# davipatti/abdpymc

Measured on NVIDIA B200. Metric: logp+grad evals/s (10k individuals, joint logp + 17-dim gradient, per chain), higher is better.
Workload: dtype f64

## Files before the change

abdpymc_b200/csrc/abd_b200.cu:

```cuda
#include <algorithm>
#include <atomic>
#include <chrono>
#include <cmath>
#include <cstdio>
#include <cstdlib>
#include <cstring>
#include <map>
#include <string>
#include <type_traits>
#include <vector>

#include <cuda_runtime.h>

#include "../../include/abd_b200.h"
#include "abd_device.cuh"

using namespace abd;

namespace {

thread_local std::string g_err;

int fail(int code, const std::string& msg) {
  g_err = msg;
// ... 181 lines not shown
    if (gap[r] < 0 || gap[r] >= G) return fail(ABD_ERR_INVALID, "gap index out of range");
    rp[(size_t)ind[r] + 1]++;
  }
  for (int n = 0; n < N; ++n) rp[n + 1] += rp[n];
  std::vector<int64_t> order((size_t)R);
  {
    std::vector<int> cur(rp.begin(), rp.end() - 1);
    for (int64_t r = 0; r < R; ++r) order[(size_t)cur[ind[r]]++] = r;
  }
  for (int n = 0; n < N; ++n)
    std::stable_sort(order.begin() + rp[n], order.begin() + rp[n + 1],
                     [&](int64_t p, int64_t q) { return gap[p] < gap[q]; });
  std::vector<double> xs((size_t)R + 2, 0.0), ods((size_t)R + 2, 0.0);
  std::vector<uint32_t> meta((size_t)R + 4, 0u);
  std::vector<uint32_t> rowcell((size_t)R + 4, 0u), cmeta;
  std::vector<int>& cp = h->h_cp[a];
  cp.assign((size_t)N + 1, 0);
  std::vector<int> perm((size_t)R);
  for (int64_t k = 0; k < R; ++k) {
    const int64_t r = order[(size_t)k];
    perm[(size_t)k] = (int)r;
    xs[(size_t)k] = x[r];
    ods[(size_t)k] = od[r];
    const uint32_t m = ((uint32_t)ind[r] << gap_bits) | (uint32_t)gap[r];
    meta[(size_t)k] = m;
    if (cmeta.empty() || cmeta.back() != m) {
      cmeta.push_back(m);
      cp[(size_t)ind[r] + 1]++;
    }
    rowcell[(size_t)k] = (uint32_t)cmeta.size() - 1;
  }
  for (int n = 0; n < N; ++n) cp[n + 1] += cp[n];
  cmeta.resize(cmeta.size() + 4, 0u);
  int rc;
  int* d_rp;
  double *d_x, *d_od;
  uint32_t *d_meta, *d_rowcell, *d_cmeta;
  if ((rc = upload(h, &d_rp, rp))) return rc;
  if ((rc = upload(h, &d_x, xs))) return rc;
  if ((rc = upload(h, &d_od, ods))) return rc;
  if ((rc = upload(h, &d_meta, meta))) return rc;
  if ((rc = upload(h, &d_rowcell, rowcell))) return rc;
  if ((rc = upload(h, &d_cmeta, cmeta))) return rc;
  {
    int* d_perm;
    if ((rc = upload(h, &d_perm, perm))) return rc;
    h->dc.rowperm[a] = d_perm;
  }
  h->dc.rcx[a] = nullptr;
  if (h->fx) {
    std::vector<uint32_t> rcx((size_t)R + 4, 0u);
    for (int64_t k = 0; k < R; ++k) {
      const double* lv = h->desc.hd.xlev;
      const int xi = (int)(std::lower_bound(lv, lv + h->desc.hd.n_xlev, xs[(size_t)k]) - lv);
      rcx[(size_t)k] = (rowcell[(size_t)k] << 5) | (uint32_t)xi;
    }
    uint32_t* d_rcx;
    if ((rc = upload(h, &d_rcx, rcx))) return rc;
    h->dc.rcx[a] = d_rcx;
  }
  h->dc.rp[a] = d_rp;
  h->dc.x[a] = d_x;
  h->dc.od[a] = d_od;
  h->dc.meta[a] = d_meta;
  h->dc.rowcell[a] = d_rowcell;
  h->dc.cmeta[a] = d_cmeta;
  return ABD_OK;
}

int get_tiling(abd_handle* h, int want, abd_handle::Tiling** out) {
  auto it = h->tilings.find(want);
  if (it == h->tilings.end()) {
    const int N = h->N;
    const std::vector<int>&rn = h->h_rp[0], &rs = h->h_rp[1];
    const double total = (double)rn[N] + (double)rs[N];
    std::vector<int> ti{0};
    int inds = 0;
    for (int n = 0; n < N; ++n) {
      const double before = (double)rn[n] + (double)rs[n];
      const double target = total * (double)ti.size() / (double)want;
      if (inds > 0 && (inds == kTileMaxInds || (before >= target && (int)ti.size() < want))) {
        ti.push_back(n);
        inds = 0;
      }
      ++inds;
    }
    ti.push_back(N);
    abd_handle::Tiling t;
    t.ntiles = (int)ti.size() - 1;
    const std::vector<int>&cn = h->h_cp[0], &cs = h->h_cp[1];
    auto span = [](int lo, int hi, int al) { return ((hi + al - 1) & ~(al - 1)) - (lo & ~(al - 1)); };
    for (int k = 0; k < t.ntiles; ++k) {
      const int a = ti[k], b = ti[k + 1];
      t.cap_n = std::max(t.cap_n, span(rn[a], rn[b], 2));
      t.cap_s = std::max(t.cap_s, span(rs[a], rs[b], 2));
      t.capr_n = std::max(t.capr_n, span(rn[a], rn[b], 4));
      t.capr_s = std::max(t.capr_s, span(rs[a], rs[b], 4));
      t.capk_n = std::max(t.capk_n, span(cn[a], cn[b], 4));
      t.capk_s = std::max(t.capk_s, span(cs[a], cs[b], 4));
    }
    t.cap_n = std::max(t.cap_n, 2);
    t.cap_s = std::max(t.cap_s, 2);
    t.capr_n = std::max(t.capr_n, 4);
    t.capr_s = std::max(t.capr_s, 4);
    t.capk_n = std::max(t.capk_n, 4);
    t.capk_s = std::max(t.capk_s, 4);
    const size_t rows_b = (size_t)(t.cap_n + t.cap_s) * 8 + (size_t)(t.capr_n + t.capr_s) * 4, cells = (size_t)(t.capk_n + t.capk_s);
    t.smem = rows_b + (h->fx ? cells * (sizeof(CellValT<true, false>) + 4)
                             : cells * (sizeof(CellValT<false, false>) + 4) + (size_t)(t.cap_n + t.cap_s) * 8);
    t.smem_cp = h->fx ? rows_b + cells * (sizeof(CellValT<true, true>) + 8 + 4) : 0;
    if (t.smem_cp && t.smem_cp + 12 * 1024 > h->smem_optin) t.smem_cp = 0;
    if (t.smem + 12 * 1024 > h->smem_optin) t.smem = 0;
    if (!t.smem && !t.smem_cp)
      return fail(ABD_ERR_INVALID, "an individual tile does not fit in shared memory (too many OD rows per 128 individuals)");
    std::vector<TileDesc> desc((size_t)t.ntiles);
    for (int k = 0; k < t.ntiles; ++k) {
      const int a = ti[k], b = ti[k + 1];
      desc[(size_t)k] = TileDesc{a, b, rn[a], rn[b], rs[a], rs[b], cn[a], cn[b], cs[a], cs[b], 0, 0};
    }
    TileDesc* d_desc = nullptr;
    int rc = upload(h, &d_desc, desc);
    if (rc) return rc;
    t.d_tiles = d_desc;
    it = h->tilings.emplace(want, t).first;
  }
  *out = &it->second;
  return ABD_OK;
}

void free_chains(abd_handle* h) {
  h->chain_bufs.release();
  if (h->h_pin) cudaFreeHost(h->h_pin);
  h->h_pin = h->h_pin_dev = nullptr;
  h->cap_chains = h->pack_valid = 0;
}

int ensure_chains(abd_handle* h, int C) {
  if (C <= 0) return fail(ABD_ERR_INVALID, "n_chains must be positive");
  if (C > 65535) return fail(ABD_ERR_INVALID, "n_chains must be <= 65535");
  if (C <= h->cap_chains) return ABD_OK;
  CU(cudaStreamSynchronize(h->stream));
  const int oldC = h->cap_chains;
  const size_t gn = (size_t)h->G * h->N;
  int rc;
  DevBufs next;
  int8_t *ni, *nw;
  if ((rc = next.alloc(&ni, (size_t)C * gn)) || (rc = next.alloc(&nw, (size_t)C * h->N))) return rc;
  CU(cudaMemset(ni, 0, (size_t)C * gn));
  CU(cudaMemset(nw, 0, (size_t)C * h->N));
  if (oldC) {
    CU(cudaMemcpy(ni, h->d_iraw, (size_t)oldC * gn, cudaMemcpyDeviceToDevice));
    CU(cudaMemcpy(nw, h->d_waner, (size_t)oldC * h->N, cudaMemcpyDeviceToDevice));
  }
  free_chains(h);
  std::swap(h->chain_bufs.ptrs, next.ptrs);
  h->d_iraw = ni;
  h->d_waner = nw;
  DevBufs& b = h->chain_bufs;
  char* pk = nullptr;
  const size_t entry = with_mask(h, [](auto m) { return sizeof(PackedState<decltype(m)>); });
  if ((rc = b.alloc(&pk, (size_t)C * h->N * entry))) return rc;
  h->d_pack = pk;
  if ((rc = b.alloc(&h->d_theta, (size_t)C * 17)) || (rc = b.alloc(&h->d_p, (size_t)C * 2)) ||
      (rc = b.alloc(&h->d_sums, (size_t)C * kNSums)) || (rc = b.alloc(&h->d_out, (size_t)C * 18)) ||
      (rc = b.alloc(&h->d_ticket, (size_t)C)) || (rc = b.alloc(&h->d_aux, (size_t)C * kAuxDoubles)) ||
      (rc = b.alloc(&h->d_traj, (size_t)C * 34)) || (rc = b.alloc(&h->d_gen, (size_t)C + 1)) ||
      (rc = b.alloc(&h->d_stats, (size_t)C * 2)) || (rc = b.alloc(&h->d_queue, (size_t)C)))
    return rc;
  CU(cudaMemset(h->d_ticket, 0, (size_t)C * sizeof(unsigned)));
  CU(cudaMemset(h->d_gen, 0, ((size_t)C + 1) * sizeof(unsigned)));
  CU(cudaMallocHost((void**)&h->h_pin, (size_t)C * 40 * sizeof(double)));
  {
    void* dp = nullptr;
    if (cudaHostGetDevicePointer(&dp, h->h_pin, 0) == cudaSuccess) h->h_pin_dev = (double*)dp;
    else cudaGetLastError();
  }
  h->cap_chains = C;
  return ABD_OK;
}

constexpr int kTileRowsOneWave = 2750;
void plan_grid(const abd_handle* h, int C, int ctas_per_sm, int cpc_fixed, int one_wave_rows, int* want_tiles,
               int* chains_per_cta) {
  const double rows = (double)(h->R[0] + h->R[1]);
  const int target = h->tile_rows_override > 0 ? h->tile_rows_override : 2200;
  const int min_tiles = (h->N + kTileMaxInds - 1) / kTileMaxInds;
  const int resident = h->n_sms * ctas_per_sm;
  auto tiles_for = [&](int cpc, int* tiles_out) -> double {
    const int groups = (C + cpc - 1) / cpc;
    int tiles = std::max(min_tiles, (int)std::ceil(rows / target));
    double waves = std::ceil((double)tiles * groups / resident);
    if ((long)tiles * groups <= 6L * resident) {
      for (int w = 1; w <= 6; ++w) {
        const int t = (resident * w) / groups;
        const double limit = (w == 1 && one_wave_rows > target && h->tile_rows_override == 0) ? (double)one_wave_rows : target * 1.02;
        if (t >= min_tiles && t >= 1 && rows / t <= limit) {
          tiles = t;
          waves = w;
          break;
        }
      }
    }
    *tiles_out = std::max(1, std::min(tiles, h->N));
    return waves;
  };
  int cpc = cpc_fixed > 0 ? cpc_fixed : (C >= 64 ? 4 : (C >= 32 ? 2 : 1));
  cpc = std::min(cpc, C);
  cpc = std::min(cpc, kMaxChainsPerCta);
  int tiles;
  const double waves1 = tiles_for(cpc, &tiles);
  if (cpc_fixed == 0 && cpc == 1 && waves1 >= 3.0) {
    double best = 9.3 * waves1;
    for (int k = 2; k <= 4 && k <= C; k *= 2) {
      if (C % k) continue;
      int tk;
      const double cost = tiles_for(k, &tk) * (1.0 + 8.3 * k);
      if (cost < 0.85 * 9.3 * waves1 && cost < best) best = cost, cpc = k, tiles = tk;
    }
  }
  *want_tiles = tiles;
  *chains_per_cta = cpc;
}

template <typename M, typename XT, bool TRAJ, bool CP>
struct SumsKernel {
  using Mask = M;
  static auto fn() { return k_sums<M, XT, TRAJ, CP>; }
};

template <typename F>
auto with_sums(const abd_handle* h, bool compact, bool traj, F&& f) {
  return with_mask(h, [&](auto m) {
    using M = decltype(m);
    if (compact) return traj ? f(SumsKernel<M, uint8_t, true, true>{}) : f(SumsKernel<M, uint8_t, false, true>{});
    if (h->fx) return traj ? f(SumsKernel<M, uint8_t, true, false>{}) : f(SumsKernel<M, uint8_t, false, false>{});
    return traj ? f(SumsKernel<M, double, true, false>{}) : f(SumsKernel<M, double, false, false>{});
  });
}

template <typename K>
cudaError_t sums_smem_attr(K, int device, size_t smem) {
  static size_t configured[64] = {};
  const int d = (device >= 0 && device < 64) ? device : 0;
  const size_t want = std::max<size_t>(smem, 48 * 1024);
  if (want <= configured[d]) return cudaSuccess;
  cudaError_t e = cudaFuncSetAttribute(K::fn(), cudaFuncAttributeMaxDynamicSharedMemorySize, (int)want);
  if (e != cudaSuccess) return e;
  e = cudaFuncSetAttribute(K::fn(), cudaFuncAttributePreferredSharedMemoryCarveout, cudaSharedmemCarveoutMaxShared);
  if (e != cudaSuccess) return e;
  configured[d] = want;
  return cudaSuccess;
}

cudaError_t sums_occupancy(const abd_handle* h, bool compact, size_t smem, int* occ) {
  return with_sums(h, compact, false, [&](auto k) {
    cudaError_t e = sums_smem_attr(k, h->device, smem);
    if (e != cudaSuccess) return e;
    return cudaOccupancyMaxActiveBlocksPerMultiprocessor(occ, decltype(k)::fn(), kSumsBlock, smem);
  });
}

cudaLaunchConfig_t pdl_config(dim3 grid, dim3 block, size_t smem, cudaStream_t st, cudaLaunchAttribute* attr) {
  cudaLaunchConfig_t lc{};
  lc.gridDim = grid;
  lc.blockDim = block;
  lc.dynamicSmemBytes = smem;
  lc.stream = st;
  attr->id = cudaLaunchAttributeProgrammaticStreamSerialization;
  attr->val.programmaticStreamSerializationAllowed = 1;
  lc.attrs = attr;
  lc.numAttrs = 1;
  return lc;
}

int resident_pack(abd_handle* h, int C, const int8_t* i_raw, const int8_t* waner, cudaStream_t st, void** out) {
  *out = nullptr;
  if (i_raw != h->d_iraw || waner != h->d_waner || !h->d_pack) return ABD_OK;
  if (h->pack_valid < C) {
    if (!h->lazy_pack) return ABD_OK;
    dim3 grid((h->N + 127) / 128, C);
    with_mask(h, [&](auto m) {
      using M = decltype(m);
      k_pack<M><<<grid, 128, 0, st>>>(h->dc, h->d_iraw, h->d_waner, (PackedState<M>*)h->d_pack);
    });
    CU(cudaGetLastError());
    h->launches++;
    h->pack_valid = C;
  }
  *out = h->d_pack;
  return ABD_OK;
}

int launch_sums(abd_handle* h, int C, const double* theta, int theta_is_q, const int8_t* i_raw,
                const int8_t* waner, double* sums, const FinalizeCfg& fin, cudaStream_t st,
                const TrajCfg* traj_in = nullptr, bool sharded = false) {
  TrajCfg traj{};
  if (traj_in) traj = *traj_in;
  const ThetaInline thin = h->thin;
  h->thin.n = 0;
  const int cpc_fixed = traj.n_steps == 1 ? 1 : h->chains_per_cta_override;
  int want, cpc, rc;
  bool compact = false;
  abd_handle::Tiling* tl = nullptr;
  for (int attempt = 0; attempt < 2 * ABD_SUMS_MINB; ++attempt) {
    const int occ = ABD_SUMS_MINB - attempt / 2;
    const int one_wave_rows = (attempt & 1) ? 0 : kTileRowsOneWave;
    plan_grid(h, C, occ, cpc_fixed, one_wave_rows, &want, &cpc);
    if (traj.n_steps > 1 && cpc != 1) {
      cpc = 1;
      want = std::max((h->N + kTileMaxInds - 1) / kTileMaxInds, (h->n_sms * occ) / C);
      want = std::max(1, std::min(want, h->N));
    }
    if ((rc = get_tiling(h, want, &tl))) return rc;
    if (tl->smem && !tl->occ) {
      int o = 0;
      CU(sums_occupancy(h, false, tl->smem, &o));
      tl->occ = std::max(o, 1);
    }
    compact = false;
    if (tl->smem && tl->occ >= occ && !(h->force_compact && tl->smem_cp)) break;
    if (tl->smem_cp && !tl->occ_cp) {
      int o = 0;
      CU(sums_occupancy(h, true, tl->smem_cp, &o));
      tl->occ_cp = std::max(o, 1);
    }
    compact = tl->smem_cp != 0;
    if (compact && tl->occ_cp >= occ) break;
  }
  const int tl_occ = compact ? tl->occ_cp : tl->occ;
  if (traj.n_steps > 1) {
    if (cpc != 1 || (long)tl->ntiles * C > (long)h->n_sms * tl_occ)
      return fail(ABD_ERR_INVALID, "abd_leapfrog_dev: too many chains for one resident grid on this cohort; "
                                   "use abd_logp_dlogp_dev per step");
  }
  const size_t need = (size_t)C * tl->ntiles * kNSums;
  if (need > h->cap_partial) {
    CU(cudaStreamSynchronize(st));
    h->partial_buf.release();
    h->cap_partial = 0;
    if ((rc = h->partial_buf.alloc(&h->d_partial, need))) return rc;
    h->cap_partial = need;
  }
  SumsCfg cfg{tl->ntiles, tl->cap_n, tl->cap_s, tl->capr_n, tl->capr_s, tl->capk_n, tl->capk_s, cpc, C};
  dim3 grid(tl->ntiles, (C + cpc - 1) / cpc);
  const size_t smem = compact ? tl->smem_cp : tl->smem;
  h->last_plan[0] = tl->ntiles, h->last_plan[1] = (int)grid.y, h->last_plan[2] = cpc;
  h->last_plan[3] = (int)smem, h->last_plan[4] = compact ? 1 : 0, h->last_plan[5] = tl_occ;
  void* pack = nullptr;
  if ((rc = resident_pack(h, C, i_raw, waner, st, &pack))) return rc;
  const bool tj = traj.n_steps > 0;
  rc = with_sums(h, compact, tj, [&](auto k) -> int {
    using K = decltype(k);
    CU(sums_smem_attr(k, h->device, smem));
    cudaLaunchAttribute attr;
    cudaLaunchConfig_t lc = pdl_config(grid, dim3(kSumsBlock), smem, st, &attr);
    if (traj.n_steps > 1) {
      int occ = 0;
      CU(cudaOccupancyMaxActiveBlocksPerMultiprocessor(&occ, K::fn(), kSumsBlock, smem));
      if ((long)grid.x * grid.y > (long)occ * h->n_sms)
        return fail(ABD_ERR_INVALID, "abd_leapfrog_dev: the grid does not fit on the device at once");
      attr.id = cudaLaunchAttributeCooperative;
      attr.val.cooperative = 1;
    }
    CU(cudaLaunchKernelEx(&lc, K::fn(), h->dc, reinterpret_cast<const TileDesc*>(tl->d_tiles), cfg, theta, theta_is_q, i_raw,
                          waner, reinterpret_cast<const PackedState<typename K::Mask>*>(pack), h->d_partial, h->d_ticket, sums,
                          fin, h->d_priors, h->d_aux, traj, sharded ? h->xch : XchCfg{}, tj ? ThetaInline{} : thin));
    return ABD_OK;
  });
  if (rc) return rc;
  CU(cudaGetLastError());
  h->launches++;
  return ABD_OK;
}

int launch_gibbs(abd_handle* h, int C, const double* theta, int theta_is_q, const double* p,
                 const double* pw, int8_t* i_raw, int8_t* waner, const GibbsCfg& cfg, cudaStream_t st) {
  if (cfg.mode == ABD_GIBBS_BLOCKED) {
    if (h->mask_bits > 32 || h->dc.ch.n < 2) {
      GibbsCfg c2 = cfg;
      c2.mode = ABD_GIBBS_HEATBATH;
      return launch_gibbs(h, C, theta, theta_is_q, p, pw, i_raw, waner, c2, st);
    }
    if (!h->gibbs_blk_ctas) {
      int occ = 0;
      CU(cudaOccupancyMaxActiveBlocksPerMultiprocessor(&occ, k_gibbs_blk, kGibbsWarps * 32, 0));
      h->gibbs_blk_ctas = h->n_sms * std::max(occ, 1);
    }
    const long items = (long)C * h->N;
    const int grid = (int)std::min<long>(h->gibbs_blk_ctas, (items + kGibbsWarps - 1) / kGibbsWarps);
    CU(cudaMemsetAsync(h->d_queue, 0, (size_t)C * sizeof(unsigned), st));
    void* pack = nullptr;
    int rcp = resident_pack(h, C, i_raw, waner, st, &pack);
    if (rcp) return rcp;
    k_gibbs_blk<<<grid, kGibbsWarps * 32, 0, st>>>(h->dc, h->d_order, C, theta, theta_is_q, p, pw, i_raw, waner,
                                                   (PackedState<uint32_t>*)pack, h->d_queue, cfg);
    CU(cudaGetLastError());
    h->launches++;
    return ABD_OK;
  }
  if (!h->gibbs_ctas) {
    int occ = 0;
    CU(with_mask(h, [&](auto m) {
      return cudaOccupancyMaxActiveBlocksPerMultiprocessor(&occ, k_gibbs<decltype(m)>, kGibbsWarps * 32, 0);
    }));
    h->gibbs_ctas = h->n_sms * std::max(occ, 1);
  }
  const long items = (long)C * h->N;
  const int grid = (int)std::min<long>(h->gibbs_ctas, (items + kGibbsWarps - 1) / kGibbsWarps);
  CU(cudaMemsetAsync(h->d_queue, 0, (size_t)C * sizeof(unsigned), st));
  void* pack = nullptr;
  int rcp = resident_pack(h, C, i_raw, waner, st, &pack);
  if (rcp) return rcp;
  with_mask(h, [&](auto m) {
    using M = decltype(m);
    k_gibbs<M><<<grid, kGibbsWarps * 32, 0, st>>>(h->dc, h->d_order, C, theta, theta_is_q, p, pw, i_raw, waner,
                                                   (PackedState<M>*)pack, h->d_queue, cfg);
  });
  CU(cudaGetLastError());
  h->launches++;
  return ABD_OK;
}

int set_device(const abd_handle* h) {
  CU(cudaSetDevice(h->device));
  return ABD_OK;
}

int copy_state(abd_handle* h, void* dst, const void* src, size_t bytes, cudaMemcpyKind dir) {
  const bool h2d = dir == cudaMemcpyHostToDevice;
  const void* host = h2d ? src : dst;
  if (bytes >= (4u << 10) && (reinterpret_cast<uintptr_t>(host) & 15u) == 0) {
    cudaPointerAttributes at{};
    if (cudaPointerGetAttributes(&at, host) == cudaSuccess && at.type == cudaMemoryTypeHost && at.devicePointer) {
      const size_t n16 = bytes / 16, rem = bytes - n16 * 16;
      const int grid = (int)std::min<size_t>((size_t)h->n_sms * 4, (n16 + 255) / 256);
      k_pull<<<grid, 256, 0, h->stream>>>(reinterpret_cast<const uint4*>(h2d ? at.devicePointer : src),
                                          reinterpret_cast<uint4*>(h2d ? dst : at.devicePointer), n16, rem);
      CU(cudaGetLastError());
      h->launches++;
      return ABD_OK;
    }
    cudaGetLastError();
  }
  CU(cudaMemcpyAsync(dst, src, bytes, dir, h->stream));
  return ABD_OK;
}

int stage_state(abd_handle* h, int C, const int8_t* i_raw, const int8_t* waner) {
  const size_t gn = (size_t)h->G * h->N;
  int rc;
  h->lazy_pack = !(i_raw || waner);
  if (i_raw || waner) h->pack_valid = 0;
  if (i_raw && (rc = copy_state(h, h->d_iraw, i_raw, (size_t)C * gn, cudaMemcpyHostToDevice))) return rc;
  if (waner && (rc = copy_state(h, h->d_waner, waner, (size_t)C * h->N, cudaMemcpyHostToDevice))) return rc;
  return ABD_OK;
}

int new_handle(abd_handle** out, int device, const CohortDesc& d) {
  abd_handle* h = new abd_handle();
  h->device = device;
  if (const char* e = std::getenv("ABD_B200_COMPACT_CELLS")) h->force_compact = (e[0] == '1');
  {
    int v = 0;
    if (cudaDeviceGetAttribute(&v, cudaDevAttrMultiProcessorCount, device) == cudaSuccess && v > 0) h->n_sms = v;
    if (cudaDeviceGetAttribute(&v, cudaDevAttrMaxSharedMemoryPerBlockOptin, device) == cudaSuccess) h->smem_optin = (size_t)v;
  }
  const CacheHeader& hd = d.hd;
  h->desc = d;
  h->G = h->dc.G = hd.G;
  h->N = h->dc.N = hd.N;
  h->mask_bits = 32 << hd.wide;
  h->R[0] = hd.R[0], h->R[1] = hd.R[1];
  h->tot = Totals{hd.tot[0], hd.tot[1], hd.tot[2], hd.tot[3]};
  h->dc.ind_offset = hd.ind_offset;
  h->dc.chain_offset = 0;
  h->dc.ch.n = hd.n_chunks;
  for (int k = 0; k < 3; ++k) h->dc.ch.mask[k] = hd.chunk_mask[k], h->dc.ch.mask_hi[k] = d.mask_hi[k];
  h->fx = hd.fx != 0;
  h->dc.n_xlev = hd.n_xlev;
  int rc = ABD_OK;
  double* d_lv = nullptr;
  if (cudaStreamCreateWithFlags(&h->stream, cudaStreamNonBlocking) != cudaSuccess) rc = fail(ABD_ERR_CUDA, "cudaStreamCreate failed");
  if (!rc) rc = upload(h, &d_lv, std::vector<double>(hd.xlev, hd.xlev + kMaxXLevels));
  if (!rc) rc = upload(h, &h->d_priors, std::vector<Priors>{default_priors(hd.G)});
  if (rc) {
    abd_destroy(h);
    return rc;
  }
  h->dc.xlev = d_lv;
  *out = h;
  return ABD_OK;
}

struct CacheIo {
  FILE* f = nullptr;
  bool writing = false, ok = true;
  ~CacheIo() {
    if (f) std::fclose(f);
  }
  void raw(void* p, size_t bytes) {
    if (!ok || !bytes) return;
    ok = writing ? std::fwrite(p, 1, bytes, f) == bytes : std::fread(p, 1, bytes, f) == bytes;
    const size_t padn = (16 - bytes % 16) % 16;
    char z[16] = {};
    if (ok && padn) ok = writing ? std::fwrite(z, 1, padn, f) == padn : std::fread(z, 1, padn, f) == padn;
  }
};

template <typename T>
int cache_array(abd_handle* h, CacheIo& io, T** dptr, size_t n, std::vector<T>* keep = nullptr) {
  std::vector<T> host(n);
  if (io.writing) {
    if (n) CU(cudaMemcpy(host.data(), *dptr, n * sizeof(T), cudaMemcpyDeviceToHost));
    io.raw(host.data(), n * sizeof(T));
  } else {
    io.raw(host.data(), n * sizeof(T));
    if (!io.ok) return fail(ABD_ERR_INVALID, "cache file truncated");
    int rc = upload(h, dptr, host);
    if (rc) return rc;
    if (keep) *keep = host;
  }
  return io.ok ? ABD_OK : fail(ABD_ERR_INVALID, "cache file I/O error");
}

int cache_body(abd_handle* h, CacheIo& io) {
  const CacheHeader& hd = h->desc.hd;
  int rc;
  const size_t N = (size_t)hd.N;
  rc = with_mask(h, [&](auto m) {
    using M = decltype(m);
    M *p = (M*)h->dc.pcr, *v = (M*)h->dc.vac;
    const int r = cache_array(h, io, &p, N);
    if (r) return r;
    h->dc.pcr = p;
    const int r2 = cache_array(h, io, &v, N);
    h->dc.vac = v;
    return r2;
  });
  if (rc) return rc;
  for (int a = 0; a < 2; ++a) {
    const size_t R = (size_t)hd.R[a], K = (size_t)hd.K[a];
    int* rp = (int*)h->dc.rp[a];
    double *x = (double*)h->dc.x[a], *od = (double*)h->dc.od[a];
    uint32_t *meta = (uint32_t*)h->dc.meta[a], *rowcell = (uint32_t*)h->dc.rowcell[a], *cmeta = (uint32_t*)h->dc.cmeta[a];
    uint32_t* rcx = (uint32_t*)h->dc.rcx[a];
    int* perm = (int*)h->dc.rowperm[a];
    if ((rc = cache_array(h, io, &perm, R))) return rc;
    h->dc.rowperm[a] = perm;
    if ((rc = cache_array(h, io, &rp, N + 1, &h->h_rp[a]))) return rc;
    if ((rc = cache_array(h, io, &x, R + 2)) || (rc = cache_array(h, io, &od, R + 2))) return rc;
    if ((rc = cache_array(h, io, &meta, R + 4)) || (rc = cache_array(h, io, &rowcell, R + 4))) return rc;
    if ((rc = cache_array(h, io, &cmeta, K + 4))) return rc;
    if (hd.fx && (rc = cache_array(h, io, &rcx, R + 4))) return rc;
    if (io.writing) {
      io.raw(h->h_cp[a].data(), (N + 1) * sizeof(int));
    } else {
      h->h_cp[a].assign(N + 1, 0);
      io.raw(h->h_cp[a].data(), (N + 1) * sizeof(int));
    }
    h->dc.rp[a] = rp, h->dc.x[a] = x, h->dc.od[a] = od, h->dc.meta[a] = meta, h->dc.rowcell[a] = rowcell;
    h->dc.cmeta[a] = cmeta, h->dc.rcx[a] = hd.fx ? rcx : nullptr;
  }
  if ((rc = cache_array(h, io, &h->d_order, N))) return rc;
  return io.ok ? ABD_OK : fail(ABD_ERR_INVALID, "cache file I/O error");
}

constexpr uint64_t kSlotUnset = 0x7FF4A5A5DEADBEEFull;
constexpr size_t kMaxPolledSlots = 18 * 64;
void unset_slots(double* ho, size_t n) {
  volatile uint64_t* slots = reinterpret_cast<volatile uint64_t*>(ho);
  for (size_t k = 0; k < n; ++k) slots[k] = kSlotUnset;
}
bool wait_slots(const double* ho, size_t n) {
  const volatile uint64_t* slots = reinterpret_cast<const volatile uint64_t*>(ho);
  const auto t0 = std::chrono::steady_clock::now();
  size_t k = 0;
  for (unsigned spins = 0; k < n; ++spins) {
    if (slots[k] != kSlotUnset) {
      ++k;
      continue;
    }
    if ((spins & 63u) == 63u && std::chrono::steady_clock::now() - t0 > std::chrono::microseconds(150)) return false;
  }
  std::atomic_thread_fence(std::memory_order_acquire);
  return true;
}

int stage_params(abd_handle* h, int C, const double* v, int k) {
  std::memcpy(h->h_pin, v, (size_t)C * k * sizeof(double));
  CU(cudaMemcpyAsync(h->d_theta, h->h_pin, (size_t)C * k * sizeof(double), cudaMemcpyHostToDevice, h->stream));
  return ABD_OK;
}

int eval_to_host(abd_handle* h, int C, const double* params, int k, double* out_val, double* out_grad, int64_t* counts) {
  int rc;
  if (C <= kInlineChains) {
    h->thin.n = C * k;
    std::memcpy(h->thin.v, params, (size_t)C * k * sizeof(double));
  } else if ((rc = stage_params(h, C, params, k))) {
    return rc;
  }
  double* ho = h->h_pin + (size_t)C * 17;
  double* dout = h->h_pin_dev ? h->h_pin_dev + (size_t)C * 17 : h->d_out;
  const FinalizeCfg fin{k == 17 ? 2 : 1, h->tot, dout, dout + C};
  const size_t nres = (size_t)C * (1 + k);
  const bool poll = h->h_pin_dev && !counts && nres <= kMaxPolledSlots;
  if (poll) unset_slots(ho, nres);
  if ((rc = launch_sums(h, C, h->d_theta, k == 17, h->d_iraw, h->d_waner, h->d_sums, fin, h->stream))) return rc;
// ... 778 lines not shown
```

abdpymc_b200/csrc/k_sums.cuh:

```cuda
#pragma once
#include "abd_kernels_common.cuh"
#include "k_nuts.cuh"

namespace {
using namespace abd;

constexpr int kInlineChains = 8;
constexpr int kMaxChainsPerCta = 32;
struct ThetaInline {
  int n;
  double v[kInlineChains * 17];
};

struct FinalizeCfg {
  int mode;
  Totals tot;
  double* out_val;
  double* out_grad;
};

struct SumsCfg {
  int ntiles;
  int cap_n, cap_s;
  int capr_n, capr_s;
  int capk_n, capk_s;
  int chains_per_cta;
  int C;
};

constexpr int kMaxPeers = 8;
constexpr unsigned long long kXchTimeoutNs = 10ull * 1000 * 1000 * 1000;
struct XchCfg {
  int world, rank, cmax;
  unsigned long long* buf[kMaxPeers];
  unsigned* seq;
  unsigned* err;
  unsigned long long* stat;
};

struct TrajCfg {
  int n_steps;
  double* q;
  double* p;
  double* grad;
  double* logp;
  const double* eps;
  const double* inv_mass;
  double* state;
  unsigned* gen;
  unsigned* err;
  NutsLeafArgs nuts;
};

struct __align__(16) TileDesc {
  int i0, i1, rn0, rn1;
  int rs0, rs1, cn0, cn1;
  int cs0, cs1, pad0, pad1;
};

template <bool FX, bool CP>
struct CellValT {
  double m, T, dT;
};
template <>
struct __align__(16) CellValT<true, false> {
  double m, T, dT, Em;
};
template <>
struct __align__(16) CellValT<true, true> {
  double T, dT;
};
constexpr int kMaxXLevels = 32;

#ifdef ABD_PHASE_TIMING
__device__ unsigned long long g_phase[4096][16];
__device__ unsigned long long g_span[256][2];
__device__ unsigned g_span_idx, g_span_done;
__device__ __forceinline__ unsigned long long gtime() {
  unsigned long long t_;
  asm volatile("mov.u64 %0, %%globaltimer;" : "=l"(t_));
  return t_;
}
#define SPAN_BEGIN()                                                                      \
  unsigned span_slot_ = 0;                                                                \
  if (threadIdx.x == 0) {                                                                 \
    span_slot_ = *(volatile unsigned*)&g_span_idx & 255u;                                 \
    atomicMin(&g_span[span_slot_][0], gtime());                                           \
  }
#define SPAN_END()                                                                        \
  if (threadIdx.x == 0) {                                                                 \
    atomicMax(&g_span[span_slot_][1], gtime());                                           \
    if (atomicAdd(&g_span_done, 1u) == gridDim.x * gridDim.y - 1) {                       \
      g_span_done = 0;                                                                    \
      __threadfence();                                                                    \
      atomicAdd(&g_span_idx, 1u);                                                         \
    }                                                                                     \
  }
#define PHASE(i)                                                                         \
  do {                                                                                   \
    if (tid == 0 && blockIdx.y * gridDim.x + blockIdx.x < 4096) {                        \
      unsigned long long t_;                                                             \
      asm volatile("mov.u64 %0, %%globaltimer;" : "=l"(t_));                             \
      g_phase[blockIdx.y * gridDim.x + blockIdx.x][i] = t_;                              \
    }                                                                                    \
  } while (0)
#define PHASEW(i, cond)                                                                  \
  do {                                                                                   \
    if ((cond) && blockIdx.y * gridDim.x + blockIdx.x < 4096) {                          \
      unsigned long long t_;                                                             \
      asm volatile("mov.u64 %0, %%globaltimer;" : "=l"(t_));                             \
      g_phase[blockIdx.y * gridDim.x + blockIdx.x][i] = t_;                              \
    }                                                                                    \
  } while (0)
#else
#define PHASE(i)
#define PHASEW(i, cond)
#define SPAN_BEGIN()
#define SPAN_END()
#endif

#ifndef ABD_ROW_UNROLL
#define ABD_ROW_UNROLL 1
#endif
#ifndef ABD_CELL_UNROLL
#define ABD_CELL_UNROLL 1
#endif
constexpr int kRowUnroll = ABD_ROW_UNROLL, kCellUnroll = ABD_CELL_UNROLL;
#ifndef ABD_SUMS_MINB
#define ABD_SUMS_MINB 3
#endif
template <typename M, typename XT, bool TRAJ, bool CP>
__global__ void __launch_bounds__(kSumsBlock, ABD_SUMS_MINB)
k_sums(const DevCohort dc, const TileDesc* __restrict__ tiles, const SumsCfg cfg,
       const double* __restrict__ theta_ptr, const int theta_is_q,
       const int8_t* __restrict__ i_raw, const int8_t* __restrict__ waner, const PackedState<M>* __restrict__ pack,
       double* __restrict__ partial, unsigned* __restrict__ ticket, double* __restrict__ sums,
       const FinalizeCfg fin, const Priors* __restrict__ priors, double* __restrict__ aux, const TrajCfg traj,
       const XchCfg xch, const __grid_constant__ ThetaInline thin) {
  const double* theta = thin.n ? thin.v : theta_ptr;
  const int tile = blockIdx.x, tid = threadIdx.x;
  const int lane = tid & 31, warp = tid >> 5;
  const int G = dc.G, N = dc.N, ntiles = cfg.ntiles;

  extern __shared__ __align__(16) unsigned char dyn_smem[];
  constexpr bool kFX = sizeof(XT) == 1;
  constexpr bool kCP = kFX && CP;
  using CellVal = CellValT<kFX, kCP>;
  double* s_od_n = reinterpret_cast<double*>(dyn_smem);
  double* s_od_s = s_od_n + cfg.cap_n;
  CellVal* s_cv_n = reinterpret_cast<CellVal*>(s_od_s + cfg.cap_s);
  CellVal* s_cv_s = s_cv_n + cfg.capk_n;
  double* s_em_n = reinterpret_cast<double*>(s_cv_s + cfg.capk_s);
  double* s_em_s = s_em_n + (kCP ? cfg.capk_n : 0);
  double* s_x_n = s_em_s + (kCP ? cfg.capk_s : 0);
  double* s_x_s = s_x_n + (kFX ? 0 : cfg.cap_n);
  uint32_t* s_rc_n = reinterpret_cast<uint32_t*>(s_x_s + (kFX ? 0 : cfg.cap_s));
  uint32_t* s_rc_s = s_rc_n + cfg.capr_n;
  uint32_t* s_cm_n = s_rc_s + cfg.capr_s;
  uint32_t* s_cm_s = s_cm_n + cfg.capk_n;

  __shared__ double s_th[16];
  __shared__ double2 s_pw[2][kGapTab<M>];
  __shared__ double s_tab[kExpTab];
  __shared__ IndState<M> s_ind[kTileMaxInds];
  __shared__ double s_red[kSumsWarps][kNSums];
  __shared__ double s_fin[kSumsBlock / 16][kNSums];
  __shared__ int s_last;
  __shared__ __align__(8) uint64_t s_bar;
  __shared__ PriorPre s_pre[17];
  __shared__ LikPre s_lik;
  __shared__ double s_q[17], s_ph[17], s_out[18];
  __shared__ double s_im[TRAJ ? 17 * 17 : 1];
  __shared__ double2 s_xe[kFX ? 2 : 1][kMaxXLevels];
  __shared__ double s_zmax[2];
  __shared__ int s_direct;

  PHASE(0);
  SPAN_BEGIN();
  griddep_launch_dependents();
  const int4 d0 = reinterpret_cast<const int4*>(tiles + tile)[0];
  const int4 d1 = reinterpret_cast<const int4*>(tiles + tile)[1];
  const int2 d2 = reinterpret_cast<const int2*>(tiles + tile)[4];
  const int i0 = d0.x, ni = d0.y - d0.x;
  const int rn0 = d0.z, rn1 = d0.w, rs0 = d1.x, rs1 = d1.y;
  const int cn0 = d1.z, cn1 = d1.w, cs0 = d2.x, cs1 = d2.y;

  const int an0 = rn0 & ~1, as0 = rs0 & ~1;
  const int qn0 = rn0 & ~3, qs0 = rs0 & ~3;
  const int kn0 = cn0 & ~3, ks0 = cs0 & ~3;
  if (tid == 0) {
    mbar_init(&s_bar, 1);
    const uint32_t bn = (uint32_t)(((rn1 + 1) & ~1) - an0) * 8u, bs = (uint32_t)(((rs1 + 1) & ~1) - as0) * 8u;
    const uint32_t bqn = (uint32_t)(((rn1 + 3) & ~3) - qn0) * 4u, bqs = (uint32_t)(((rs1 + 3) & ~3) - qs0) * 4u;
    const uint32_t bkn = (uint32_t)(((cn1 + 3) & ~3) - kn0) * 4u, bks = (uint32_t)(((cs1 + 3) & ~3) - ks0) * 4u;
    mbar_expect_tx(&s_bar, (kFX ? bn + bs : 2 * bn + 2 * bs) + bqn + bqs + bkn + bks);
    if (bkn) bulk_g2s(s_cm_n, dc.cmeta[0] + kn0, bkn, &s_bar);
    if (bks) bulk_g2s(s_cm_s, dc.cmeta[1] + ks0, bks, &s_bar);
    if (bn) {
      bulk_g2s(s_od_n, dc.od[0] + an0, bn, &s_bar);
      if (!kFX) bulk_g2s(s_x_n, dc.x[0] + an0, bn, &s_bar);
    }
    if (bs) {
      bulk_g2s(s_od_s, dc.od[1] + as0, bs, &s_bar);
      if (!kFX) bulk_g2s(s_x_s, dc.x[1] + as0, bs, &s_bar);
    }
    if (bqn) bulk_g2s(s_rc_n, (kFX ? dc.rcx[0] : dc.rowcell[0]) + qn0, bqn, &s_bar);
    if (bqs) bulk_g2s(s_rc_s, (kFX ? dc.rcx[1] : dc.rowcell[1]) + qs0, bqs, &s_bar);
  }
  fill_exp_table(s_tab, tid, kSumsBlock);
  M my_pcr = 0, my_vac = 0;
  if (tid < ni) {
    my_pcr = reinterpret_cast<const M*>(dc.pcr)[i0 + tid];
    my_vac = reinterpret_cast<const M*>(dc.vac)[i0 + tid];
  }
  double x_lev = 0.0;
  if (kFX && warp == kSumsWarps - 1) x_lev = dc.xlev[lane];
  __syncthreads();
  griddep_wait();
  if (TRAJ) {
    for (int k = tid; k < 17 * 17; k += kSumsBlock) s_im[k] = traj.inv_mass[k];
    __syncthreads();
  }
  PHASE(1);

  __shared__ int s_pend[kMaxChainsPerCta], s_npend;
  __shared__ unsigned s_pend_seq[kMaxChainsPerCta];
  __shared__ unsigned s_xw[kMaxPeers][32];
  if (tid == 0) s_npend = 0;
  auto load_aux = [&](int c) {
    if (fin.mode && tid < kAuxDoubles) {
      const double v = __ldcg(aux + (size_t)c * kAuxDoubles + tid);
      if (tid < 17 * 7) reinterpret_cast<double*>(s_pre)[tid] = v;
      else if (tid < 17 * 7 + 6) reinterpret_cast<double*>(&s_lik)[tid - 17 * 7] = v;
    }
  };
  auto sum_partials = [&](int c, bool sharded_) {
    const int k = tid & 15, g = tid >> 4;
    double v = 0.0;
    const double* src = partial + (size_t)c * ntiles * kNSums + k;
    for (int tl = g; tl < ntiles; tl += 8 * (kSumsBlock / 16)) {
      double ld[8];
#pragma unroll
      for (int u = 0; u < 8; ++u) {
        const int tt = tl + u * (kSumsBlock / 16);
        ld[u] = __ldcg(src + (size_t)min(tt, ntiles - 1) * kNSums);
      }
#pragma unroll
      for (int u = 0; u < 8; ++u) v += (tl + u * (kSumsBlock / 16) < ntiles) ? ld[u] : 0.0;
    }
    s_fin[g][k] = v;
    PHASE(9);
    __syncthreads();
    if (tid < kNSums) {
      double tot = 0.0;
#pragma unroll
      for (int gg = 0; gg < kSumsBlock / 16; ++gg) tot += s_fin[gg][tid];
      s_red[0][tid] = tot;
      if (sums && !sharded_) sums[(size_t)c * kNSums + tid] = tot;
    }
    if (tid == 0) ticket[c] = 0;
    __syncthreads();
  };
  unsigned tk_prev = 0;
  int tk_c = 0;
  bool tk_valid = false;
  auto finalize_chain = [&](int c, int step, int nsteps) {
    if (fin.mode == 1) {
      if (lane == 0)
        finalize_loglik_post(s_th, s_lik, s_red[0], fin.tot, &fin.out_val[c],
                             fin.out_grad ? &fin.out_grad[(size_t)c * 13] : nullptr);
    } else if (fin.mode == 2 && !TRAJ) {
      finalize_logp_post(lane, s_pre, s_th, s_lik, s_red[0], fin.tot, &fin.out_val[c],
                         fin.out_grad ? &fin.out_grad[(size_t)c * 17] : nullptr);
    } else if (TRAJ && fin.mode == 2) {
      finalize_logp_post(lane, s_pre, s_th, s_lik, s_red[0], fin.tot, &s_out[0], &s_out[1]);
      __syncwarp();
      const double e = traj.eps[c];
      const double g = lane < 17 ? s_out[1 + lane] : 0.0;
      const double ph = lane < 17 ? s_ph[lane] : 0.0;
      if (step == nsteps - 1) {
        if (lane < 17) {
          traj.q[(size_t)c * 17 + lane] = s_q[lane];
          traj.p[(size_t)c * 17 + lane] = fma(0.5 * e, g, ph);
          traj.grad[(size_t)c * 17 + lane] = g;
        }
        if (lane == 0) traj.logp[c] = s_out[0];
        if (traj.nuts.state) {
          __syncwarp();
          nuts_leaf_chain(traj.nuts, c, lane, traj.q, traj.p, traj.grad, traj.logp, s_im);
        }
      } else {
        const double ph2 = fma(e, g, ph);
        double dot = 0.0;
        for (int j = 0; j < 17; ++j) {
          const double pj = __shfl_sync(0xffffffffu, ph2, j);
          if (lane < 17) dot = fma(s_im[lane * 17 + j], pj, dot);
        }
        if (lane < 17) {
          traj.state[(size_t)c * 34 + lane] = fma(e, dot, s_q[lane]);
          traj.state[(size_t)c * 34 + 17 + lane] = ph2;
        }
        __threadfence();
        __syncwarp();
        if (lane == 0) {
          const unsigned nxt = (unsigned)step + 1u;
          asm volatile("st.release.gpu.u32 [%0], %1;" ::"l"(traj.gen + c), "r"(nxt) : "memory");
        }
      }
    }
  };

  for (int cc = 0; cc < cfg.chains_per_cta; ++cc) {
    const int c = blockIdx.y * cfg.chains_per_cta + cc;
    if (c >= cfg.C) break;

    const int nsteps = TRAJ ? traj.n_steps : 1;
    double cnt_i = 0.0, cnt_w = 0.0;
    if (tid < ni && pack) {
      const PackedState<M> ps = pack[(size_t)c * N + i0 + tid];
      const M w = ps.rw & top_bit<M>();
      IndState<M> st;
      st.inf = ps.inf;
      st.vacw = my_vac | w;
      s_ind[tid] = st;
      cnt_i = (double)popc(ps.rw & ~top_bit<M>());
      cnt_w = w ? 1.0 : 0.0;
    } else if (tid < ni) {
      const M raw = load_column<M>(i_raw + (size_t)c * G * N + i0 + tid, G, N);
      const int w = waner[(size_t)c * N + i0 + tid] != 0;
      IndState<M> st;
      st.inf = constrain<M>(raw, my_pcr, dc.ch);
      st.vacw = my_vac | (w ? top_bit<M>() : (M)0);
      s_ind[tid] = st;
      cnt_i = (double)popc(raw);
      cnt_w = (double)w;
    }
    for (int step = 0; step < nsteps; ++step) {
    double acc[kNSums];
#pragma unroll
    for (int k = 0; k < kNSums; ++k) acc[k] = 0.0;
    acc[S_KI] = cnt_i;
    acc[S_KW] = cnt_w;

    double q_lane = 0.0, ph_lane = 0.0;
    if (TRAJ) {
      if (step > 0) {
        if (tid == 0) {
          unsigned seen, polls = 0;
          do {
            asm volatile("ld.acquire.gpu.u32 %0, [%1];" : "=r"(seen) : "l"(traj.gen + c) : "memory");
          } while (seen < (unsigned)step && ++polls < (1u << 26));
          if (seen < (unsigned)step) *traj.err = 1u;
        }
        __syncthreads();
        if (lane < 17) {
          q_lane = __ldcg(traj.state + (size_t)c * 34 + lane);
          ph_lane = __ldcg(traj.state + (size_t)c * 34 + 17 + lane);
        }
      } else if (warp >= 4) {
        const double e = traj.eps[c];
        double mine = 0.0;
        if (lane < 17) mine = fma(0.5 * e, traj.grad[(size_t)c * 17 + lane], traj.p[(size_t)c * 17 + lane]);
        double dot = 0.0;
        for (int j = 0; j < 17; ++j) {
          const double pj = __shfl_sync(0xffffffffu, mine, j);
          if (lane < 17) dot = fma(s_im[lane * 17 + j], pj, dot);
        }
        ph_lane = mine;
        if (lane < 17) q_lane = fma(e, dot, traj.q[(size_t)c * 17 + lane]);
      }
    }
    auto param13 = [&](int k13) -> double {
      if (TRAJ) {
        const int j = kQOfTheta[k13];
        return backward(__shfl_sync(0xffffffffu, q_lane, j), kQTransform[j]);
      }
      return load_param(theta, theta_is_q, c, k13);
    };

    if (tid < kTileMaxInds) {
      PHASEW(12, tid == 0);
    } else if (warp == 4) {
      fill_pow2_warp(param13(N_RHO), G, lane, s_pw[0]);
      PHASEW(13, lane == 0);
    } else if (warp == 5) {
      fill_pow2_warp(param13(S_RHO), G, lane, s_pw[1]);
    } else if (warp == 6) {
      if (TRAJ) {
        const int j = kQOfTheta[lane < 13 ? lane : 0];
        const double v = backward(__shfl_sync(0xffffffffu, q_lane, j), kQTransform[j]);
        if (lane < 13) s_th[lane] = v;
      } else if (lane < 13) {
        s_th[lane] = load_param(theta, theta_is_q, c, lane);
      }
      PHASEW(14, lane == 0);
    } else if (warp == kSumsWarps - 1) {
      if (kFX) {
        const double zn = -param13(N_B) * x_lev, zs = -param13(S_B) * x_lev;
        double mn = (lane < dc.n_xlev) ? fabs(zn) : 0.0, ms = (lane < dc.n_xlev) ? fabs(zs) : 0.0;
#pragma unroll
        for (int off = 16; off > 0; off >>= 1) {
          mn = fmax(mn, __shfl_xor_sync(0xffffffffu, mn, off));
          ms = fmax(ms, __shfl_xor_sync(0xffffffffu, ms, off));
        }
        const bool direct = !(mn < 300.0 && ms < 300.0);
        s_xe[0][lane] = make_double2(x_lev, direct ? 0.0 : fast_exp(zn, s_tab));
        s_xe[kFX ? 1 : 0][lane] = make_double2(x_lev, direct ? 0.0 : fast_exp(zs, s_tab));
        if (lane == 0) {
          s_zmax[0] = 700.0 - mn;
          s_zmax[1] = 700.0 - ms;
          s_direct = direct;
        }
      }
      if (TRAJ && lane < 17) {
        s_q[lane] = q_lane;
        s_ph[lane] = ph_lane;
      }
      PHASEW(15, lane == 0);
    }
    __syncthreads();
    PHASE(2);
    const bool aux_cta = (tile == 0);
    const int nwork = aux_cta ? kSumsBlock - 32 : kSumsBlock;
    if (aux_cta && fin.mode != 0 && warp == kSumsWarps - 1) {
      double* a = aux + (size_t)c * kAuxDoubles;
      if (fin.mode == 2 && lane < 17) {
        const PriorPre pp = prior_pre(lane, TRAJ ? s_q[lane] : theta[(size_t)c * 17 + lane], priors->v[lane]);
        double* o = a + lane * 7;
        o[0] = pp.lpA, o[1] = pp.dA, o[2] = pp.f, o[3] = pp.lx, o[4] = pp.l1mx, o[5] = pp.x, o[6] = pp.omx;
      }
      if (lane == 17) {
        const LikPre lk = lik_pre(s_th[N_SIGMA], s_th[S_SIGMA]);
        double* o = a + 17 * 7;
        o[0] = lk.lsn, o[1] = lk.lss, o[2] = lk.ivn, o[3] = lk.ivs, o[4] = lk.isn, o[5] = lk.iss;
      }
    }
    if (cc == 0 && step == 0) mbar_wait(&s_bar, 0);
    PHASE(3);

    {
      const double init = s_th[N_INIT], perm = s_th[N_PERM], temp = s_th[N_TEMP];
      const double bn_fx = s_th[N_B], zmax_n = s_zmax[0];
#pragma unroll kCellUnroll
      for (int k = cn0 + tid; k < cn1 && tid < nwork; k += nwork) {
        const uint32_t mt = s_cm_n[k - kn0];
        const int t = mt & kGapMask<M>, li = (int)(mt >> kGapBits<M>) - i0;
        double P, T, dT;
        traj_n<M>(s_ind[li].inf, t, s_pw[0], P, T, dT);
        CellVal cv;
        const double m = init + perm * P + temp * T;
        cv.T = T;
        cv.dT = (P != 0.0) ? dT : -0.0;
        if constexpr (!kCP) cv.m = m;
        if constexpr (kFX) {
          const double z = bn_fx * m;
          const double em = fast_exp((z > zmax_n) ? zmax_n : z, s_tab);
          if constexpr (kCP) s_em_n[k - cn0] = em;
          else cv.Em = em;
        }
        s_cv_n[k - cn0] = cv;
      }
    }
    {
      const double init = s_th[S_INIT], perm = s_th[S_PERM];
      const double bs_fx = s_th[S_B], zmax_s = s_zmax[1];
#pragma unroll kCellUnroll
      for (int k = cs0 + tid; k < cs1 && tid < nwork; k += nwork) {
        const uint32_t mt = s_cm_s[k - ks0];
        const int t = mt & kGapMask<M>, li = (int)(mt >> kGapBits<M>) - i0;
        const IndState<M> st = s_ind[li];
        double P, U, dU;
        traj_s<M>(st.inf, st.vacw & ~top_bit<M>(), (st.vacw & top_bit<M>()) != 0, t, s_pw[1], P, U, dU);
        CellVal cv;
        const double m = init + perm * P + U;
        cv.T = kCP ? m : U;
        cv.dT = (P != 0.0) ? dU : -0.0;
        if constexpr (!kCP) cv.m = m;
        if constexpr (kFX) {
          const double z = bs_fx * m;
          const double em = fast_exp((z > zmax_s) ? zmax_s : z, s_tab);
          if constexpr (kCP) s_em_s[k - cs0] = em;
          else cv.Em = em;
        }
        s_cv_s[k - cs0] = cv;
      }
    }
    __syncthreads();
    PHASE(4);

    auto rows = [&](auto direct_tag) {
      [[maybe_unused]] constexpr bool kDirect = decltype(direct_tag)::value;
      {
        const double b = s_th[N_B], d = s_th[N_D];
        const uint32_t* rcp = s_rc_n - qn0;
        const double* odp = s_od_n - an0;
        const CellVal* cvp = s_cv_n - cn0;
        [[maybe_unused]] const double* emp = s_em_n - cn0;
#pragma unroll kRowUnroll
        for (int r = rn0 + tid; r < rn1 && tid < nwork; r += nwork) {
          double sg, res, q, xm;
          const uint32_t rc = rcp[r];
          const CellVal cv = cvp[kFX ? (rc >> 5) : rc];
          if constexpr (kCP) {
            const double2 xe = s_xe[0][rc & 31];
            if constexpr (kDirect) {
              const double m = s_th[N_INIT] + ((__double2hiint(cv.dT) < 0) ? 0.0 : s_th[N_PERM]) + s_th[N_TEMP] * cv.T;
              row_eval(xe.x, odp[r], m, b, d, s_tab, sg, res, q, xm);
            } else {
              row_eval_E(xe.y * emp[rc >> 5], odp[r], d, sg, res, q);
              xm = xe.x;
            }
          } else if constexpr (kFX) {
            const double2 xe = s_xe[0][rc & 31];
            xm = xe.x - cv.m;
            if constexpr (kDirect) row_eval(xe.x, odp[r], cv.m, b, d, s_tab, sg, res, q, xm);
            else row_eval_E(xe.y * cv.Em, odp[r], d, sg, res, q);
          } else {
            row_eval((s_x_n - an0)[r], odp[r], cv.m, b, d, s_tab, sg, res, q, xm);
          }
          acc[SN_0] = fma(res, res, acc[SN_0]);
          acc[SN_1] = fma(res, sg, acc[SN_1]);
          acc[SN_2] = fma(q, xm, acc[SN_2]);
          acc[SN_QINIT] += q;
          acc[SN_QPERM] += (__double2hiint(cv.dT) < 0) ? 0.0 : q;
          acc[SN_QTEMP] = fma(q, cv.T, acc[SN_QTEMP]);
          acc[SN_QRHO] = fma(q, cv.dT, acc[SN_QRHO]);
        }
      }
      {
        const double b = s_th[S_B], d = s_th[S_D];
        const uint32_t* rcp = s_rc_s - qs0;
        const double* odp = s_od_s - as0;
        const CellVal* cvp = s_cv_s - cs0;
        [[maybe_unused]] const double* emp = s_em_s - cs0;
#pragma unroll kRowUnroll
        for (int r = rs0 + tid; r < rs1 && tid < nwork; r += nwork) {
          double sg, res, q, xm;
          const uint32_t rc = rcp[r];
          const CellVal cv = cvp[kFX ? (rc >> 5) : rc];
          if constexpr (kCP) {
            const double2 xe = s_xe[1][rc & 31];
            xm = xe.x - cv.T;
            if constexpr (kDirect) row_eval(xe.x, odp[r], cv.T, b, d, s_tab, sg, res, q, xm);
            else row_eval_E(xe.y * emp[rc >> 5], odp[r], d, sg, res, q);
          } else if constexpr (kFX) {
            const double2 xe = s_xe[1][rc & 31];
            xm = xe.x - cv.m;
            if constexpr (kDirect) row_eval(xe.x, odp[r], cv.m, b, d, s_tab, sg, res, q, xm);
            else row_eval_E(xe.y * cv.Em, odp[r], d, sg, res, q);
          } else {
            row_eval((s_x_s - as0)[r], odp[r], cv.m, b, d, s_tab, sg, res, q, xm);
          }
          acc[SS_0] = fma(res, res, acc[SS_0]);
          acc[SS_1] = fma(res, sg, acc[SS_1]);
          acc[SS_2] = fma(q, xm, acc[SS_2]);
          acc[SS_QINIT] += q;
          acc[SS_QPERM] += (__double2hiint(cv.dT) < 0) ? 0.0 : q;
          acc[SS_QRHO] = fma(q, cv.dT, acc[SS_QRHO]);
        }
      }
    };
    if (!kFX || s_direct) rows(std::true_type{});
    else rows(std::false_type{});

    PHASE(5);
    {
      const double tot = warp_reduce16(acc, lane);
      if ((lane & 1) == 0) s_red[warp][warp_reduce16_index(lane)] = tot;
    }
    __syncthreads();
    if (warp == 0) {
      double v = 0.0;
      if (lane < kNSums) {
#pragma unroll
        for (int wv = 0; wv < kSumsWarps; ++wv) v += s_red[wv][lane];
      }
      if constexpr (kCP) {
        if (!s_direct) {
          const double qi = __shfl_sync(0xffffffffu, v, SN_QINIT), qp = __shfl_sync(0xffffffffu, v, SN_QPERM);
          const double qt = __shfl_sync(0xffffffffu, v, SN_QTEMP);
          if (lane == SN_2) v -= s_th[N_INIT] * qi + s_th[N_PERM] * qp + s_th[N_TEMP] * qt;
        }
      }
      if (lane < kNSums) partial[((size_t)c * ntiles + tile) * kNSums + lane] = v;
    }

    PHASE(6);
    __syncthreads();
    if (!((TRAJ && nsteps > 1) || (cfg.chains_per_cta == 1 && xch.world <= 1))) {
      if (tid == 0) {
        if (tk_valid && tk_prev == (unsigned)(ntiles - 1)) s_pend[s_npend++] = tk_c;
        asm volatile("atom.add.acq_rel.gpu.global.u32 %0, [%1], 1;" : "=r"(tk_prev) : "l"(ticket + c) : "memory");
        tk_c = c;
        tk_valid = true;
      }
      PHASE(8);
      continue;
    }
    if (tid == 0) {
      unsigned prev;
      asm volatile("atom.add.acq_rel.gpu.global.u32 %0, [%1], 1;" : "=r"(prev) : "l"(ticket + c) : "memory");
      s_last = (prev == (unsigned)(ntiles - 1));
    }
    __syncthreads();
    PHASE(7);
    if (s_last) {
      load_aux(c);
      sum_partials(c, false);
      PHASE(10);
      if (warp == 0) finalize_chain(c, step, nsteps);
    }
    if (s_last) PHASE(11);
    PHASE(8);
    __syncthreads();
    }
  }

  if (tid == 0 && tk_valid && tk_prev == (unsigned)(ntiles - 1)) s_pend[s_npend++] = tk_c;
  __syncthreads();
  const int npend = s_npend;
  const bool sharded = xch.world > 1;
  PHASE(7);
  for (int pi = 0; pi < npend; ++pi) {
    const int c = s_pend[pi];
    if (!sharded) {
      load_aux(c);
      if (!TRAJ && warp == 1 && lane < 13) s_th[lane] = load_param(theta, theta_is_q, c, lane);
    }
    sum_partials(c, sharded);
    PHASE(10);
    if (!sharded) {
      if (warp == 0) finalize_chain(c, 0, 1);
      __syncthreads();
      continue;
    }
    const unsigned seq = xch.seq[c] + 1u;
    if (tid < 32 * xch.world) {
      const int r = tid >> 5, j = tid & 31;
      const double val = s_red[0][j >> 1];
      const unsigned half = (j & 1) ? (unsigned)__double2hiint(val) : (unsigned)__double2loint(val);
      const unsigned long long word = ((unsigned long long)seq << 32) | half;
      unsigned long long* dst = xch.buf[r] + ((((size_t)(seq & 1u) * xch.world + xch.rank) * xch.cmax + c) << 5) + j;
      asm volatile("st.relaxed.sys.global.u64 [%0], %1;" ::"l"(dst), "l"(word) : "memory");
    }
    __syncthreads();
    if (tid == 0) {
      xch.seq[c] = seq;
      s_pend_seq[pi] = seq;
    }
  }
  if (npend) PHASE(11);

  if (sharded) {
    __syncthreads();
    for (int pi = 0; pi < npend; ++pi) {
      const int c = s_pend[pi];
      const unsigned seq = s_pend_seq[pi];
      load_aux(c);
      if (!TRAJ && warp == 0 && lane < 13) s_th[lane] = load_param(theta, theta_is_q, c, lane);
      if (tid < 32 * xch.world) {
        const int r = tid >> 5, j = tid & 31;
        const unsigned long long* mine = xch.buf[xch.rank] + ((((size_t)(seq & 1u) * xch.world + r) * xch.cmax + c) << 5) + j;
        unsigned long long word, t_start, t_now;
        asm volatile("mov.u64 %0, %%globaltimer;" : "=l"(t_start));
        do {
          asm volatile("ld.relaxed.sys.global.u64 %0, [%1];" : "=l"(word) : "l"(mine) : "memory");
          asm volatile("mov.u64 %0, %%globaltimer;" : "=l"(t_now));
        } while ((unsigned)(word >> 32) != seq && t_now - t_start < kXchTimeoutNs);
        if ((unsigned)(word >> 32) != seq) *xch.err = 1u;
        s_xw[r][j] = (unsigned)word;
        if (j == 0) {
          atomicAdd(xch.stat + r, t_now - t_start);
          if (r == 0) atomicAdd(xch.stat + kMaxPeers, 1ull);
        }
      }
      __syncthreads();
      if (tid < kNSums) {
        double tot = 0.0;
        for (int r = 0; r < xch.world; ++r) tot += __hiloint2double((int)s_xw[r][2 * tid + 1], (int)s_xw[r][2 * tid]);
        s_red[0][tid] = tot;
        if (sums) sums[(size_t)c * kNSums + tid] = tot;
      }
      __syncthreads();
      if (warp == 0) finalize_chain(c, 0, 1);
      __syncthreads();
    }
  }
  SPAN_END();
}

__global__ void k_finalize(const int C, const double* __restrict__ theta,
                           const double* __restrict__ sums, const FinalizeCfg fin,
                           const Priors* __restrict__ priors) {
  const int c = (blockIdx.x * blockDim.x + threadIdx.x) >> 5, lane = threadIdx.x & 31;
  if (c >= C) return;
  if (fin.mode == 1) {
    if (lane == 0)
      finalize_loglik(&theta[(size_t)c * 13], &sums[(size_t)c * kNSums], fin.tot, &fin.out_val[c],
                      fin.out_grad ? &fin.out_grad[(size_t)c * 13] : nullptr);
  } else {
    __shared__ double s_th[4][16];
    __shared__ PriorPre s_pre[4][17];
    const int wv = threadIdx.x >> 5;
    if (lane < 13) s_th[wv][lane] = load_param(theta, 1, c, lane);
    if (lane < 17) s_pre[wv][lane] = prior_pre(lane, theta[(size_t)c * 17 + lane], priors->v[lane]);
    __syncwarp();
    finalize_logp_post(lane, s_pre[wv], s_th[wv], lik_pre(s_th[wv][N_SIGMA], s_th[wv][S_SIGMA]),
                       &sums[(size_t)c * kNSums], fin.tot, &fin.out_val[c],
                       fin.out_grad ? &fin.out_grad[(size_t)c * 17] : nullptr);
  }
}

}
```

Baseline: 338,900.

## Raise non-trajectory sums occupancy, widen partial gather, trim register state

The launch bound of the sums kernel now depends on the template: the non-trajectory variant asks for four resident blocks per SM instead of three, and the host-side occupancy search follows the same function. The cross-tile partial reduction issues more loads per iteration in the non-trajectory path to hide latency. Several per-thread values move out of registers: x_lev goes to shared memory, xch becomes a grid constant, and the ticket bookkeeping drops tk_c and tk_valid by deriving the chain index. The start index of the second cell loop is also rotated so threads that finished the first loop pick up work evenly. The tighter register budget may cause spills, and the derived pending-chain index assumes chains are visited consecutively.

```diff
diff --git a/abdpymc_b200/csrc/abd_b200.cu b/abdpymc_b200/csrc/abd_b200.cu
--- a/abdpymc_b200/csrc/abd_b200.cu
+++ b/abdpymc_b200/csrc/abd_b200.cu
@@ -507,8 +507,9 @@
   int want, cpc, rc;
   bool compact = false;
   abd_handle::Tiling* tl = nullptr;
-  for (int attempt = 0; attempt < 2 * ABD_SUMS_MINB; ++attempt) {
-    const int occ = ABD_SUMS_MINB - attempt / 2;
+  const int occ_max = sums_min_blocks(traj.n_steps > 0);
+  for (int attempt = 0; attempt < 2 * occ_max; ++attempt) {
+    const int occ = occ_max - attempt / 2;
     const int one_wave_rows = (attempt & 1) ? 0 : kTileRowsOneWave;
     plan_grid(h, C, occ, cpc_fixed, one_wave_rows, &want, &cpc);
     if (traj.n_steps > 1 && cpc != 1) {
diff --git a/abdpymc_b200/csrc/k_sums.cuh b/abdpymc_b200/csrc/k_sums.cuh
--- a/abdpymc_b200/csrc/k_sums.cuh
+++ b/abdpymc_b200/csrc/k_sums.cuh
@@ -126,17 +126,17 @@
 #define ABD_CELL_UNROLL 1
 #endif
 constexpr int kRowUnroll = ABD_ROW_UNROLL, kCellUnroll = ABD_CELL_UNROLL;
-#ifndef ABD_SUMS_MINB
-#define ABD_SUMS_MINB 3
-#endif
+constexpr int sums_min_blocks(bool traj) { return traj ? 3 : 4; }
+template <bool TRAJ>
+constexpr int kGatherLoads = TRAJ ? 8 : 19;
 template <typename M, typename XT, bool TRAJ, bool CP>
-__global__ void __launch_bounds__(kSumsBlock, ABD_SUMS_MINB)
+__global__ void __launch_bounds__(kSumsBlock, sums_min_blocks(TRAJ))
 k_sums(const DevCohort dc, const TileDesc* __restrict__ tiles, const SumsCfg cfg,
        const double* __restrict__ theta_ptr, const int theta_is_q,
        const int8_t* __restrict__ i_raw, const int8_t* __restrict__ waner, const PackedState<M>* __restrict__ pack,
        double* __restrict__ partial, unsigned* __restrict__ ticket, double* __restrict__ sums,
        const FinalizeCfg fin, const Priors* __restrict__ priors, double* __restrict__ aux, const TrajCfg traj,
-       const XchCfg xch, const __grid_constant__ ThetaInline thin) {
+       const __grid_constant__ XchCfg xch, const __grid_constant__ ThetaInline thin) {
   const double* theta = thin.n ? thin.v : theta_ptr;
   const int tile = blockIdx.x, tid = threadIdx.x;
   const int lane = tid & 31, warp = tid >> 5;
@@ -213,8 +213,11 @@
     my_pcr = reinterpret_cast<const M*>(dc.pcr)[i0 + tid];
     my_vac = reinterpret_cast<const M*>(dc.vac)[i0 + tid];
   }
-  double x_lev = 0.0;
-  if (kFX && warp == kSumsWarps - 1) x_lev = dc.xlev[lane];
+  if (kFX && warp == kSumsWarps - 1) {
+    const double x_lev = dc.xlev[lane];
+    s_xe[0][lane].x = x_lev;
+    s_xe[kFX ? 1 : 0][lane].x = x_lev;
+  }
   __syncthreads();
   griddep_wait();
   if (TRAJ) {
@@ -238,15 +241,15 @@
     const int k = tid & 15, g = tid >> 4;
     double v = 0.0;
     const double* src = partial + (size_t)c * ntiles * kNSums + k;
-    for (int tl = g; tl < ntiles; tl += 8 * (kSumsBlock / 16)) {
-      double ld[8];
+    for (int tl = g; tl < ntiles; tl += kGatherLoads<TRAJ> * (kSumsBlock / 16)) {
+      double ld[kGatherLoads<TRAJ>];
 #pragma unroll
-      for (int u = 0; u < 8; ++u) {
+      for (int u = 0; u < kGatherLoads<TRAJ>; ++u) {
         const int tt = tl + u * (kSumsBlock / 16);
         ld[u] = __ldcg(src + (size_t)min(tt, ntiles - 1) * kNSums);
       }
 #pragma unroll
-      for (int u = 0; u < 8; ++u) v += (tl + u * (kSumsBlock / 16) < ntiles) ? ld[u] : 0.0;
+      for (int u = 0; u < kGatherLoads<TRAJ>; ++u) v += (tl + u * (kSumsBlock / 16) < ntiles) ? ld[u] : 0.0;
     }
     s_fin[g][k] = v;
     PHASE(9);
@@ -262,8 +265,7 @@
     __syncthreads();
   };
   unsigned tk_prev = 0;
-  int tk_c = 0;
-  bool tk_valid = false;
+  const bool defer_ticket = !((TRAJ && traj.n_steps > 1) || (cfg.chains_per_cta == 1 && xch.world <= 1));
   auto finalize_chain = [&](int c, int step, int nsteps) {
     if (fin.mode == 1) {
       if (lane == 0)
@@ -396,6 +398,7 @@
       PHASEW(14, lane == 0);
     } else if (warp == kSumsWarps - 1) {
       if (kFX) {
+        const double x_lev = s_xe[0][lane].x;
         const double zn = -param13(N_B) * x_lev, zs = -param13(S_B) * x_lev;
         double mn = (lane < dc.n_xlev) ? fabs(zn) : 0.0, ms = (lane < dc.n_xlev) ? fabs(zs) : 0.0;
 #pragma unroll
@@ -404,8 +407,8 @@
           ms = fmax(ms, __shfl_xor_sync(0xffffffffu, ms, off));
         }
         const bool direct = !(mn < 300.0 && ms < 300.0);
-        s_xe[0][lane] = make_double2(x_lev, direct ? 0.0 : fast_exp(zn, s_tab));
-        s_xe[kFX ? 1 : 0][lane] = make_double2(x_lev, direct ? 0.0 : fast_exp(zs, s_tab));
+        s_xe[0][lane].y = direct ? 0.0 : fast_exp(zn, s_tab);
+        s_xe[kFX ? 1 : 0][lane].y = direct ? 0.0 : fast_exp(zs, s_tab);
         if (lane == 0) {
           s_zmax[0] = 700.0 - mn;
           s_zmax[1] = 700.0 - ms;
@@ -464,8 +467,9 @@
     {
       const double init = s_th[S_INIT], perm = s_th[S_PERM];
       const double bs_fx = s_th[S_B], zmax_s = s_zmax[1];
+      const int s_first = (tid + nwork - (cn1 - cn0) % nwork) % nwork;
 #pragma unroll kCellUnroll
-      for (int k = cs0 + tid; k < cs1 && tid < nwork; k += nwork) {
+      for (int k = cs0 + s_first; k < cs1 && tid < nwork; k += nwork) {
         const uint32_t mt = s_cm_s[k - ks0];
         const int t = mt & kGapMask<M>, li = (int)(mt >> kGapBits<M>) - i0;
         const IndState<M> st = s_ind[li];
@@ -587,12 +591,10 @@
 
     PHASE(6);
     __syncthreads();
-    if (!((TRAJ && nsteps > 1) || (cfg.chains_per_cta == 1 && xch.world <= 1))) {
+    if (defer_ticket) {
       if (tid == 0) {
-        if (tk_valid && tk_prev == (unsigned)(ntiles - 1)) s_pend[s_npend++] = tk_c;
+        if (cc > 0 && tk_prev == (unsigned)(ntiles - 1)) s_pend[s_npend++] = c - 1;
         asm volatile("atom.add.acq_rel.gpu.global.u32 %0, [%1], 1;" : "=r"(tk_prev) : "l"(ticket + c) : "memory");
-        tk_c = c;
-        tk_valid = true;
       }
       PHASE(8);
       continue;
@@ -616,7 +618,8 @@
     }
   }
 
-  if (tid == 0 && tk_valid && tk_prev == (unsigned)(ntiles - 1)) s_pend[s_npend++] = tk_c;
+  if (tid == 0 && defer_ticket && tk_prev == (unsigned)(ntiles - 1))
+    s_pend[s_npend++] = min((int)(blockIdx.y + 1) * cfg.chains_per_cta, cfg.C) - 1;
   __syncthreads();
   const int npend = s_npend;
   const bool sharded = xch.world > 1;
```

After: 345,400, median of 6. 1.9% higher.
